# anthonyhu/tumblr-emotions

Hardware: AMD Instinct MI355X
Metric: training samples/sec (224x224 img + 32-tok text, batch 256) (higher is better)
Workload: dtype f32; 1 GPU; joint train step (fwd+bwd+all-reduce+Adam): Inception-v1 224x224x3 + 300-d embedding + LSTM-512, T=32, V=10000, 15 classes, batch 256 per GPU, reference freeze (<=Mixed_5b conv weights frozen, all BN betas trainable), dropout 0.8, BN train mode; global_batch=256, per_gpu_batch=256, parallelism=dp1, launch=eager

## Files before the change

### tumblr_emotions_amd/csrc/conv_igemm.hip

```cpp
#include <stdlib.h>
#include <mutex>
#include <type_traits>
#include <unordered_map>
#include "conv_epilogue.h"

using ds::f32x16;
typedef float f32x4 __attribute__((ext_vector_type(4)));
typedef float f32x2 __attribute__((ext_vector_type(2)));
typedef unsigned int u32x4 __attribute__((ext_vector_type(4)));
typedef __attribute__((address_space(3))) void *lds_ptr;

namespace {

constexpr int BK = 16;
constexpr int LDK = 20;
using ds::kOOB;
using ds::make_srd;

struct ConvParams {
    ds_conv_desc d;
    const float *x;
    const float *w;
    float *z;
    const float *bias;
// ... 772 lines not shown
                                                       srd_w, (okn && kk + 1 < d.Cin) ? (off + (unsigned)d.w_k_stride) * 4u : kOOB, 0, 0));
            }
        } else {
#pragma unroll
            for (int i = 0; i < BJ; ++i) {
                const int nn = n0 + srow + 32 * i;
                const bool ok = nn < d.Cout && k < d.Cin;
                const unsigned off = wt + (unsigned)nn * (unsigned)d.w_n_stride + (unsigned)k;
                rb[i] = __builtin_bit_cast(f32x4, __builtin_amdgcn_raw_buffer_load_b128(srd_w, ok ? off * 4u : kOOB, 0, 0));
            }
        }
        ++tap;
        if (++dw == d.KW) {
            dw = 0;
            if (++dh == d.KH) { dh = 0; tap = 0; c0 += HK; }
        }
    };

    auto store_tile = [&](int buf) {
        __bf16 *a_s = As + buf * BM * HLD;
        __bf16 *b_s = Bs + buf * BN * HLD;
#pragma unroll
        for (int j = 0; j < AJ; ++j)
            *reinterpret_cast<bf16x4 *>(a_s + (srow + 32 * j) * HLD + c4) = __builtin_convertvector(ra[j], bf16x4);
        if (BNMAJOR) {
#pragma unroll
            for (int i = 0; i < BP; ++i) {
                const int pi = tid + 256 * i;
                const int kp = pi / (BN / 4), n4 = pi - kp * (BN / 4);
                if (pi < 4 * BN) {
#pragma unroll
                    for (int jj = 0; jj < 4; ++jj) {
                        const f32x2 pr = {rb[2 * i][jj], rb[2 * i + 1][jj]};
                        *reinterpret_cast<bf16x2 *>(b_s + (4 * n4 + jj) * HLD + 2 * kp) = __builtin_convertvector(pr, bf16x2);
                    }
                }
            }
        } else {
#pragma unroll
            for (int i = 0; i < BJ; ++i)
                *reinterpret_cast<bf16x4 *>(b_s + (srow + 32 * i) * HLD + c4) = __builtin_convertvector(rb[i], bf16x4);
        }
    };

    auto compute = [&](int buf) {
        const __bf16 *a_s = As + buf * BM * HLD + (wm * 32 + li) * HLD + kh * 8;
        const __bf16 *b_s = Bs + buf * BN * HLD + li * HLD + kh * 8;
#pragma unroll
        for (int ks = 0; ks < 2; ++ks) {
            const bf16x8 a = *reinterpret_cast<const bf16x8 *>(a_s + ks * 16);
#pragma unroll
            for (int b = 0; b < NT; ++b) {
                const bf16x8 w = *reinterpret_cast<const bf16x8 *>(b_s + b * 32 * HLD + ks * 16);
                acc[b] = __builtin_amdgcn_mfma_f32_32x32x16_bf16(a, w, acc[b], 0, 0, 0);
            }
        }
    };

    int par = 0;
    if (tid0.row < p.row_tiles) {
        setup_tile(tid0.row);
        load_tile();
        store_tile(0);
    }
    __syncthreads();
    for (int tile = tid0.row; tile < p.row_tiles; tile += tid0.stride) {
        const int m0 = tile * BM;
        const bool has_next = tile + tid0.stride < p.row_tiles;
#pragma unroll
        for (int b = 0; b < NT; ++b)
#pragma unroll
            for (int r = 0; r < 16; ++r) acc[b][r] = 0.f;
        for (int kt = 0; kt < KT; ++kt) {
            const bool last = kt + 1 == KT;
            if (last && has_next) setup_tile(tile + tid0.stride);
            const bool fetch = !last || has_next;
            if (fetch) load_tile();
            compute(par);
            if (fetch) store_tile(par ^ 1);
            __syncthreads();
            par ^= 1;
        }
#pragma unroll
        for (int b = 0; b < NT; ++b) {
            const int col = n0 + b * 32 + li;
            const bool colok = col < d.Cout;
            const float bv = ((flags & DS_EPI_BIAS) && colok) ? p.bias[col] : 0.f;
            const float pv = (p.pivot && colok) ? p.pivot[col] : 0.f;
            float s = 0.f, q = 0.f;
#pragma unroll
            for (int r = 0; r < 16; ++r) {
                const int row = m0 + wm * 32 + (r & 3) + 8 * (r >> 2) + 4 * kh;
                if (row < p.M && colok) {
                    float v = acc[b][r] + bv;
                    const int64_t off = (int64_t)row * d.ldz + col;
                    if (flags & DS_EPI_ACCUM) v += zout[off];
                    if (flags & DS_EPI_MASK) v = p.mask[(int64_t)row * d.ldmask + col] > 0.f ? v : 0.f;
                    if (flags & DS_EPI_RELU) v = fmaxf(v, 0.f);
                    zout[off] = v;
                    const float u = v - pv;
                    s += u;
                    q += u * u;
                }
            }
            csum[b] += s;
            csq[b] += q;
        }
    }

    if (flags & DS_EPI_STATS) {
        float *red = reinterpret_cast<float *>(smem);
        __syncthreads();
#pragma unroll
        for (int b = 0; b < NT; ++b) {
            const float s = csum[b] + __shfl_xor(csum[b], 32);
            const float q = csq[b] + __shfl_xor(csq[b], 32);
            if (kh == 0) {
                const int c = b * 32 + li;
                red[(wm * BN + c) * 2 + 0] = s;
                red[(wm * BN + c) * 2 + 1] = q;
            }
        }
        __syncthreads();
        if (tid < BN && n0 + tid < d.Cout && tid0.row < p.row_tiles) {
            float s = 0.f, q = 0.f;
#pragma unroll
            for (int w = 0; w < 4; ++w) {
                s += red[(w * BN + tid) * 2 + 0];
                q += red[(w * BN + tid) * 2 + 1];
            }
            p.stats[(int64_t)(n0 + tid) * tid0.stride + tid0.row] = s;
            p.stats[((int64_t)d.Cout + n0 + tid) * tid0.stride + tid0.row] = q;
        }
    }
}


#ifndef DS_WIDE_A_B2B
#define DS_WIDE_A_B2B 1
#endif
template <int N>
__device__ __forceinline__ void barrier_keep_vm() { asm volatile("s_waitcnt vmcnt(%0) lgkmcnt(0)\n\ts_barrier" ::"n"(N) : "memory"); }

template <bool BNR>
struct WideEpi : ds::WaveRowOpt { static constexpr bool bnr = BNR, mask_rstd = true, publish = true; };

template <int NB, bool BNMAJOR, bool BNB = false, bool POOL = false, int AST = 0, bool BNR = false>
__global__ __launch_bounds__(256, NB <= 4 ? 3 : 2) void gemm_wide_kernel(const ConvParams p) {
    constexpr int BN = NB * 32, WK = 16;
    constexpr int DJ = (WK * BN / 4 + 255) / 256;
    constexpr int BSZ = DJ * 1024;
    constexpr int BST = AST > 0 ? AST - 1 : 2;
    static_assert(AST == 0 || (AST >= 3 && !BNB && !POOL), "the A ring is built for the plain and the normalising loader");
    __shared__ __attribute__((aligned(128))) float smem[BST * BSZ + 256 + AST * 2048];
    __shared__ __attribute__((aligned(16))) float nrm[BNB ? 5 : 2][1024 + WK];
    const ds_conv_desc &d = p.d;
    const int tid = threadIdx.x, lane = tid & 63;
    const int wave = __builtin_amdgcn_readfirstlane(tid >> 6);
    const int li = lane & 31, kh = lane >> 5;
    const TileId t0 = tile_id(p);
    const int n0 = t0.col * BN;
    const bool item = t0.row < p.row_tiles;
    const __amdgpu_buffer_rsrc_t srd_x = make_srd(p.x, p.x_bytes);
    const __amdgpu_buffer_rsrc_t srd_w = make_srd(p.w, p.w_bytes);
    const int K = d.Cin;
    int mrow0 = t0.row * 128 + wave * 32, Mw = p.M;
    bool hasU = false, hasD = false, hasL = false, hasR = false;
    int prow = 0;
    if constexpr (POOL) {
        const int blk = t0.row * 4 + wave;
        const int n = blk / p.pool_bpi, rb = blk - n * p.pool_bpi;
        const int r0 = rb * p.pool_rpb;
        const int rows = (d.H - r0) < p.pool_rpb ? (d.H - r0) : p.pool_rpb;
        const int cnt = (item && n < d.N) ? rows * d.W : 0;
        mrow0 = (n * d.H + r0) * d.W;
        Mw = mrow0 + cnt;
        const int dr = li / d.W, ow = li - dr * d.W, oh = r0 + dr;
        const bool ok = li < cnt;
        hasU = ok && oh > 0;
        hasD = ok && oh + 1 < d.H;
        hasL = ok && ow > 0;
        hasR = ok && ow + 1 < d.W;
        prow = d.W * d.ldx * 4;
    }
    const int m = mrow0 + li;
    const unsigned voff = (item && m < Mw) ? ((unsigned)m * (unsigned)d.ldx + 4u * kh) * 4u : kOOB;

    unsigned uoff[DJ];
    int ukq[DJ];
#pragma unroll
    for (int i = 0; i < DJ; ++i) {
        const int idx = i * 256 + tid;
        if (BNMAJOR) {
            const int k = idx / (BN / 4), n = n0 + (idx % (BN / 4)) * 4;
            ukq[i] = k;
            uoff[i] = (n < d.Cout && k < WK) ? ((unsigned)k * (unsigned)d.w_k_stride + (unsigned)n) * 4u : kOOB;
        } else {
            const int nl = idx >> 2, pc = idx & 3, kq = pc ^ ((nl >> 2) & 3);
            ukq[i] = kq * 4;
            uoff[i] = (n0 + nl < d.Cout && nl < BN) ? ((unsigned)(n0 + nl) * (unsigned)d.w_n_stride + 4u * kq) * 4u : kOOB;
        }
    }
    auto dma_b = [&](int buf, int c0, int i) {
        const bool ok = c0 + ukq[i] < K;
        const unsigned off = BNMAJOR ? uoff[i] + (unsigned)c0 * (unsigned)d.w_k_stride * 4u : uoff[i] + (unsigned)c0 * 4u;
        unsigned o = off;
        if (!ok || uoff[i] == 0x80000000u) o = 0x80000000u;
        __builtin_amdgcn_raw_ptr_buffer_load_lds(srd_w, (lds_ptr)(smem + buf * BSZ + wave * 256 + i * 1024), 16, o, 0, 0, 0);
    };

    f32x16 acc[NB];
#pragma unroll
    for (int b = 0; b < NB; ++b)
#pragma unroll
        for (int e = 0; e < 16; ++e) acc[b][e] = 0.f;

    const unsigned vup = (POOL && hasU) ? voff - (unsigned)prow : kOOB, vdn = (POOL && hasD) ? voff + (unsigned)prow : kOOB;
    const __amdgpu_buffer_rsrc_t srd_am = make_srd(POOL ? (const void *)d.pool_argmax : (const void *)p.x,
                                                   POOL ? (unsigned)((int64_t)p.M * K) : 0u);
    const unsigned vam = (POOL && item && m < Mw && t0.col == 0) ? (unsigned)m * (unsigned)K + 4u * kh : kOOB;
    f32x4 ru0, ru1, rd0, rd1;
    auto load_ud = [&](int c0) {
        ru0 = __builtin_bit_cast(f32x4, __builtin_amdgcn_raw_buffer_load_b128(srd_x, vup, c0 * 4, 0));
        ru1 = __builtin_bit_cast(f32x4, __builtin_amdgcn_raw_buffer_load_b128(srd_x, vup, c0 * 4 + 32, 0));
        rd0 = __builtin_bit_cast(f32x4, __builtin_amdgcn_raw_buffer_load_b128(srd_x, vdn, c0 * 4, 0));
        rd1 = __builtin_bit_cast(f32x4, __builtin_amdgcn_raw_buffer_load_b128(srd_x, vdn, c0 * 4 + 32, 0));
    };
    auto from_left = [](float v) -> float {
        return __builtin_bit_cast(float, __builtin_amdgcn_update_dpp(0, __builtin_bit_cast(int, v), 0x138 , 0xf, 0xf, false));
    };
    auto from_right = [](float v) -> float {
        return __builtin_bit_cast(float, __builtin_amdgcn_update_dpp(0, __builtin_bit_cast(int, v), 0x130 , 0xf, 0xf, false));
    };
    auto pool4 = [&](f32x4 &c, const f32x4 &u, const f32x4 &dn) -> unsigned {
        unsigned bytes = 0;
#pragma unroll
        for (int j = 0; j < 4; ++j) {
            const float uu = hasU ? u[j] : -INFINITY, dd = hasD ? dn[j] : -INFINITY;
            const float cm = fmaxf(fmaxf(uu, c[j]), dd);
            const int t = uu == cm ? 0 : (c[j] == cm ? 3 : 6);
            const float lraw = from_left(cm), rraw = from_right(cm);
            const int tl = __builtin_amdgcn_update_dpp(0, t, 0x138, 0xf, 0xf, false);
            const int tr = __builtin_amdgcn_update_dpp(0, t, 0x130, 0xf, 0xf, false);
            const float lv = hasL ? lraw : -INFINITY, rv = hasR ? rraw : -INFINITY;
            const float best = fmaxf(fmaxf(lv, cm), rv);
            const int il = lv == best ? tl : 99, ic = cm == best ? t + 1 : 99, ir = rv == best ? tr + 2 : 99;
            const int arg = min(min(il, ic), ir);
            c[j] = best;
            bytes |= (unsigned)arg << (8 * j);
        }
        return bytes;
    };
    f32x4 a0 = {0.f, 0.f, 0.f, 0.f}, a1 = {0.f, 0.f, 0.f, 0.f};
    if constexpr (AST == 0) {
        a0 = __builtin_bit_cast(f32x4, __builtin_amdgcn_raw_buffer_load_b128(srd_x, voff, 0, 0));
        a1 = __builtin_bit_cast(f32x4, __builtin_amdgcn_raw_buffer_load_b128(srd_x, voff, 32, 0));
    }
    if constexpr (POOL) load_ud(0);
    const ds_bn_bwd_on_load &bb = p.bnb;
    __amdgpu_buffer_rsrc_t srd_dy[3];
    unsigned vdy[3];
    if (BNB) {
#pragma unroll
        for (int sg = 0; sg < 3; ++sg) {
            const bool has = sg < bb.nseg;
            const int cb = sg == 0 ? 0 : bb.c_end[sg - 1];
            const int ld = has ? bb.ld[sg] : 0;
            srd_dy[sg] = make_srd(has ? bb.dy[sg] : bb.dy[0], has ? (unsigned)(((int64_t)(p.M - 1) * ld + (bb.c_end[sg] - cb)) * 4) : 0u);
            vdy[sg] = (has && item && m < p.M) ? ((unsigned)m * (unsigned)ld + 4u * kh) * 4u : kOOB;
        }
    }
    auto load_dy = [&](int c0, int half) -> f32x4 {
        const int sg = (c0 < bb.c_end[0] || bb.nseg == 1) ? 0 : ((c0 < bb.c_end[1] || bb.nseg == 2) ? 1 : 2);
        const int cb = sg == 0 ? 0 : bb.c_end[sg - 1];
        const __amdgpu_buffer_rsrc_t r = sg == 0 ? srd_dy[0] : (sg == 1 ? srd_dy[1] : srd_dy[2]);
        const unsigned v = sg == 0 ? vdy[0] : (sg == 1 ? vdy[1] : vdy[2]);
        return __builtin_bit_cast(f32x4, __builtin_amdgcn_raw_buffer_load_b128(r, v, (c0 - cb) * 4 + 32 * half, 0));
    };
    f32x4 d0 = {0.f, 0.f, 0.f, 0.f}, d1 = {0.f, 0.f, 0.f, 0.f};
    if (BNB) {
        d0 = load_dy(0, 0);
        d1 = load_dy(0, 1);
    }
    if constexpr (AST == 0) {
#pragma unroll
        for (int i = 0; i < DJ; ++i) dma_b(0, 0, i);
    }
    const int ksteps = (K + WK - 1) / WK;
    const bool norm = d.norm_rstd != nullptr;
    if (norm) {
        for (int c = tid; c < ksteps * WK; c += 256) {
            nrm[0][c] = c < K ? d.norm_rstd[c] : 0.f;
            nrm[1][c] = c < K ? d.norm_shift[c] : 0.f;
        }
    }
    auto apply_norm = [&](f32x4 &a, int c) {
        const f32x4 r = *reinterpret_cast<const f32x4 *>(&nrm[0][c]), sh = *reinterpret_cast<const f32x4 *>(&nrm[1][c]);
        const f32x4 zero = {0.f, 0.f, 0.f, 0.f};
        a = __builtin_elementwise_max(__builtin_elementwise_fma(a, r, sh), zero);
    };
    if (BNB) {
        for (int c = tid; c < ksteps * WK; c += 256) {
            nrm[0][c] = c < K ? bb.rstd[c] : 0.f;
            nrm[1][c] = c < K ? bb.shift[c] : 0.f;
            nrm[BNB ? 2 : 0][c] = c < K ? bb.mean[c] : 0.f;
            nrm[BNB ? 3 : 0][c] = c < K ? bb.coef[c] : 0.f;
            nrm[BNB ? 4 : 0][c] = c < K ? bb.coef[K + c] : 0.f;
        }
    }
    auto apply_bnb = [&](f32x4 &a, const f32x4 &dy, int c) {
        const f32x4 r = *reinterpret_cast<const f32x4 *>(&nrm[0][c]), sh = *reinterpret_cast<const f32x4 *>(&nrm[1][c]);
        const f32x4 mu = *reinterpret_cast<const f32x4 *>(&nrm[BNB ? 2 : 0][c]);
        const f32x4 k1 = *reinterpret_cast<const f32x4 *>(&nrm[BNB ? 3 : 0][c]), k2 = *reinterpret_cast<const f32x4 *>(&nrm[BNB ? 4 : 0][c]);
#pragma unroll
        for (int j = 0; j < 4; ++j) a[j] = ds::bn_bwd_dz(a[j], dy[j], r[j], sh[j], mu[j], k1[j], k2[j]);
    };
    __syncthreads();
    auto pool_step = [&](int c0) {
        const unsigned w0 = pool4(a0, ru0, rd0), w1 = pool4(a1, ru1, rd1);
        __builtin_amdgcn_raw_buffer_store_b32(w0, srd_am, vam, c0, 0);
        __builtin_amdgcn_raw_buffer_store_b32(w1, srd_am, vam, c0 + 8, 0);
    };
    if constexpr (POOL) pool_step(0);
    if (norm && AST == 0) {
        apply_norm(a0, 4 * kh);
        apply_norm(a1, 8 + 4 * kh);
    }
    if (BNB) {
        apply_bnb(a0, d0, 4 * kh);
        apply_bnb(a1, d1, 8 + 4 * kh);
    }
    if constexpr (AST > 0) {
        float *const ring = smem + BST * BSZ + 256;
        unsigned aoff[2];
#pragma unroll
        for (int j = 0; j < 2; ++j) {
            const int row = 16 * j + (lane >> 2), chunk = (lane & 3) ^ ((row >> 1) & 3);
            const int mr = mrow0 + row;
            aoff[j] = (item && mr < Mw) ? ((unsigned)mr * (unsigned)d.ldx + 4u * chunk) * 4u : kOOB;
        }
        auto dma_a = [&](int stage, int c0) {
#pragma unroll
            for (int j = 0; j < 2; ++j)
                __builtin_amdgcn_raw_ptr_buffer_load_lds(srd_x, (lds_ptr)(ring + (stage * 4 + wave) * 512 + j * 256), 16, aoff[j], c0 * 4, 0, 0);
        };
        auto dma_b_all = [&](int buf, int c0) {
#pragma unroll
            for (int i = 0; i < DJ; ++i) dma_b(buf, c0, i);
        };
#pragma unroll
        for (int j = -(AST - 1); j < 0; ++j) {
            if (j + AST - 2 >= 0 && j + AST - 2 < ksteps) dma_b_all((j + AST - 2) % BST, (j + AST - 2) * WK);
            if (j + AST - 1 < ksteps) dma_a((j + AST - 1) % AST, (j + AST - 1) * WK);
        }
        constexpr int KEEP = 2 * (AST - 2) + DJ * (AST - 3);
        if (ksteps > AST - 1) barrier_keep_vm<KEEP>(); else barrier_keep_vm<0>();
        int bst = 0, ast = 0;
        const int swz = (li >> 1) & 3;
        for (int ks = 0; ks < ksteps; ++ks) {
            const float *ra = ring + (ast * 4 + wave) * 512 + li * 16;
            a0 = *reinterpret_cast<const f32x4 *>(ra + ((kh ^ swz) * 4));
            a1 = *reinterpret_cast<const f32x4 *>(ra + (((2 + kh) ^ swz) * 4));
            if (norm) {
                apply_norm(a0, ks * WK + 4 * kh);
                apply_norm(a1, ks * WK + 8 + 4 * kh);
            }
            const float *b_s = smem + bst * BSZ;
#pragma unroll
            for (int b = 0; b < NB; ++b) {
                float bf[8];
                if (BNMAJOR) {
#pragma unroll
                    for (int j = 0; j < 4; ++j) {
                        bf[j] = b_s[(4 * kh + j) * BN + 32 * b + li];
                        bf[4 + j] = b_s[(8 + 4 * kh + j) * BN + 32 * b + li];
                    }
                } else {
                    const int nl = 32 * b + li, sw = (nl >> 2) & 3;
                    const f32x4 lo = *reinterpret_cast<const f32x4 *>(b_s + nl * 16 + ((kh ^ sw) * 4));
                    const f32x4 hi = *reinterpret_cast<const f32x4 *>(b_s + nl * 16 + (((2 + kh) ^ sw) * 4));
#pragma unroll
                    for (int j = 0; j < 4; ++j) { bf[j] = lo[j]; bf[4 + j] = hi[j]; }
                }
                if (b == 0) {
                    if (ks + AST - 2 < ksteps) dma_b_all((bst + AST - 2) % BST, (ks + AST - 2) * WK);
                    if (ks + AST - 1 < ksteps) dma_a((ast + AST - 1) % AST, (ks + AST - 1) * WK);
                }
                __builtin_amdgcn_sched_barrier(0);
#pragma unroll
                for (int j = 0; j < 4; ++j) acc[b] = __builtin_amdgcn_mfma_f32_32x32x2f32(a0[j], bf[j], acc[b], 0, 0, 0);
#pragma unroll
                for (int j = 0; j < 4; ++j) acc[b] = __builtin_amdgcn_mfma_f32_32x32x2f32(a1[j], bf[4 + j], acc[b], 0, 0, 0);
                __builtin_amdgcn_sched_barrier(0);
            }
            if (ks + AST - 1 < ksteps) barrier_keep_vm<KEEP>(); else barrier_keep_vm<0>();
            bst = bst + 1 == BST ? 0 : bst + 1;
            ast = ast + 1 == AST ? 0 : ast + 1;
        }
    }
    for (int ks = 0; AST == 0 && ks < ksteps; ++ks) {
        const bool more = ks + 1 < ksteps;
        const int cn = (ks + 1) * WK;
        const float *b_s = smem + (ks & 1) * BSZ;
        f32x4 n0v = a0, n1v = a1;
#pragma unroll
        for (int b = 0; b < NB; ++b) {
            float bf[8];
            if (BNMAJOR) {
#pragma unroll
                for (int j = 0; j < 4; ++j) {
                    bf[j] = b_s[(4 * kh + j) * BN + 32 * b + li];
                    bf[4 + j] = b_s[(8 + 4 * kh + j) * BN + 32 * b + li];
                }
            } else {
                const int nl = 32 * b + li, sw = (nl >> 2) & 3;
                const f32x4 lo = *reinterpret_cast<const f32x4 *>(b_s + nl * 16 + ((kh ^ sw) * 4));
                const f32x4 hi = *reinterpret_cast<const f32x4 *>(b_s + nl * 16 + (((2 + kh) ^ sw) * 4));
#pragma unroll
                for (int j = 0; j < 4; ++j) { bf[j] = lo[j]; bf[4 + j] = hi[j]; }
            }
            if (more) {
                if (b == 0) {
                    n0v = __builtin_bit_cast(f32x4, __builtin_amdgcn_raw_buffer_load_b128(srd_x, voff, cn * 4, 0));
                    if (BNB) d0 = load_dy(cn, 0);
                }
                if (b == ((NB > 1 && !DS_WIDE_A_B2B) ? 1 : 0)) {
                    n1v = __builtin_bit_cast(f32x4, __builtin_amdgcn_raw_buffer_load_b128(srd_x, voff, cn * 4 + 32, 0));
                    if (BNB) d1 = load_dy(cn, 1);
                    if constexpr (POOL) load_ud(cn);
                }
                if (b < DJ) dma_b((ks + 1) & 1, cn, b);
            }
            __builtin_amdgcn_sched_barrier(0);
#pragma unroll
            for (int j = 0; j < 4; ++j) acc[b] = __builtin_amdgcn_mfma_f32_32x32x2f32(a0[j], bf[j], acc[b], 0, 0, 0);
#pragma unroll
            for (int j = 0; j < 4; ++j) acc[b] = __builtin_amdgcn_mfma_f32_32x32x2f32(a1[j], bf[4 + j], acc[b], 0, 0, 0);
            __builtin_amdgcn_sched_barrier(0);
        }
        if (more && DJ > NB) {
#pragma unroll
            for (int i = NB; i < DJ; ++i) dma_b((ks + 1) & 1, cn, i);
        }
        a0 = n0v;
        a1 = n1v;
        if constexpr (POOL) {
            if (more) pool_step(cn);
        }
        if (norm && more) {
            apply_norm(a0, cn + 4 * kh);
            apply_norm(a1, cn + 8 + 4 * kh);
        }
        if (BNB && more) {
            apply_bnb(a0, d0, cn + 4 * kh);
            apply_bnb(a1, d1, cn + 8 + 4 * kh);
        }
        __syncthreads();
    }

    const int flags = d.flags;
    float *red = smem + BST * BSZ;
    ds::wave_row_epilogue<NB, WideEpi<BNR>>(acc, d, p.z, p.mask, p.stats, p.pivot, item, n0, mrow0, Mw, Mw > mrow0, t0.row, t0.stride,
                                            red, wave, li, kh, p.scale, p.shift, p.fin.ticket != nullptr);
    if (p.fin.ticket && item && (flags & DS_EPI_STATS)) {
        __builtin_amdgcn_s_waitcnt(0);
        __syncthreads();
        if (tid == 0) {
            const unsigned old = __hip_atomic_fetch_add(p.fin.ticket + t0.col, 1u, __ATOMIC_RELAXED, __HIP_MEMORY_SCOPE_AGENT);
            red[0] = old + 1 == (unsigned)p.row_tiles ? 1.f : 0.f;
        }
        __syncthreads();
        if (red[0] != 0.f) {
            const int cend = min(n0 + BN, d.Cout);
            for (int c = n0 + wave; c < cend; c += 4)
                ds::bn_finalize_channel_by_wave(p.stats, t0.stride, d.Cout, c, p.fin_inv_count, p.fin, p.pivot);
            if (tid == 0) __hip_atomic_store(p.fin.ticket + t0.col, 0u, __ATOMIC_RELAXED, __HIP_MEMORY_SCOPE_AGENT);
        }
    }
}


struct Bf16dEpi : ds::WaveRowOpt { static constexpr bool half = true, mask_rstd = true; };

template <int NB, int KS, bool XB, bool X3 = false>
__global__ __launch_bounds__(256, 2) void conv_bf16d_kernel(const ConvParams p) {
    constexpr int BN = NB * 32, SI = !X3 ? 4 : NB == 1 ? 4 : NB <= 4 ? 2 : 1, TAPS = KS * KS;
    constexpr int PL = X3 ? 3 : 1;
    constexpr int NSL = SI * PL * NB / 4;
    static_assert(SI * PL * NB % 4 == 0, "a step's weight tile must be whole 256-lane DMA instructions");
    constexpr int BSZ = SI * PL * BN * 16;
    static_assert(!(X3 && XB), "ds_conv_f32x3 reads fp32 activations");
    __shared__ __attribute__((aligned(128))) __bf16 smem[2 * BSZ + 512];
    __shared__ __attribute__((aligned(16))) float nrm[2][X3 ? 1024 + 16 : 4];
    const ds_conv_desc &d = p.d;
    const int tid = threadIdx.x, lane = tid & 63;
    const int wave = __builtin_amdgcn_readfirstlane(tid >> 6);
    const int li = lane & 31, kh = lane >> 5;
    const TileId t0 = tile_id(p);
    const int n0 = t0.col * BN;
    const bool item = t0.row < p.row_tiles;
    const __amdgpu_buffer_rsrc_t srd_x = make_srd(p.x, p.x_bytes);
    const __amdgpu_buffer_rsrc_t srd_w = make_srd(p.w, p.w_bytes);
    const int chunks = (d.Cin + 15) >> 4;
    const int iters = chunks * TAPS;
    const int nsteps = (iters + SI - 1) / SI;

    const int m = t0.row * 128 + wave * 32 + li;
    const bool rv = item && m < p.M;
    const int ohw = d.OH * d.OW;
    const int n = (rv ? m : 0) / ohw;
    const int r = (rv ? m : 0) - n * ohw;
    const int oh = r / d.OW, ow = r - oh * d.OW;
    unsigned voff[TAPS];
#pragma unroll
    for (int a = 0; a < KS; ++a)
#pragma unroll
        for (int b = 0; b < KS; ++b) {
            const int ih = oh * d.stride - d.pad_t + a, iw = ow * d.stride - d.pad_l + b;
            const bool ok = rv && (unsigned)ih < (unsigned)d.H && (unsigned)iw < (unsigned)d.W;
            voff[a * KS + b] = ok ? ((unsigned)((n * d.H + ih) * d.W + iw) * (unsigned)d.ldx + 8u * kh) * (XB ? 2u : 4u) : kOOB;
        }
    const int ncols = p.col_total;
    unsigned uoff[NSL];
    int uit[NSL];
#pragma unroll
    for (int i = 0; i < NSL; ++i) {
        const int sl = i * 256 + tid;
        const int itl = sl / (BN * 2), nn = (sl >> 1) % BN, half = sl & 1;
        uit[i] = itl;
        uoff[i] = (n0 + nn < ncols) ? ((unsigned)((itl * ncols + n0 + nn) * 16 + 8 * half)) * 2u : kOOB;
    }
    const unsigned it_bytes = (unsigned)ncols * 32u;
    auto dma_b = [&](int buf, int step, int i) {
        unsigned o = uoff[i] + (unsigned)(step * SI * PL) * it_bytes;
        if (step * SI * PL + uit[i] >= iters * PL || uoff[i] == 0x80000000u) o = 0x80000000u;
        __builtin_amdgcn_raw_ptr_buffer_load_lds(srd_w, (lds_ptr)(smem + buf * BSZ + wave * 512 + i * 2048), 16, o, 0, 0, 0);
    };
    auto load_a = [&](int it, f32x4 &lo, f32x4 &hi) {
        const int chunk = it / TAPS, tap = it - chunk * TAPS;
        unsigned vo = voff[0];
#pragma unroll
        for (int k = 1; k < TAPS; ++k) vo = tap == k ? voff[k] : vo;
        if (XB) {
            lo = __builtin_bit_cast(f32x4, __builtin_amdgcn_raw_buffer_load_b128(srd_x, vo, chunk * 32, 0));
        } else {
            lo = __builtin_bit_cast(f32x4, __builtin_amdgcn_raw_buffer_load_b128(srd_x, vo, chunk * 64, 0));
            hi = __builtin_bit_cast(f32x4, __builtin_amdgcn_raw_buffer_load_b128(srd_x, vo, chunk * 64 + 16, 0));
        }
    };

    f32x16 acc[NB];
#pragma unroll
    for (int b = 0; b < NB; ++b)
#pragma unroll
        for (int e = 0; e < 16; ++e) acc[b][e] = 0.f;

    f32x4 alo[SI], ahi[SI];
#pragma unroll
    for (int j = 0; j < SI; ++j) load_a(j, alo[j], ahi[j]);
#pragma unroll
    for (int i = 0; i < NSL; ++i) dma_b(0, 0, i);
    bool norm = false;
    if constexpr (X3) {
        norm = d.norm_rstd != nullptr;
        if (norm)
            for (int c = tid; c < chunks * 16; c += 256) {
                nrm[0][c] = c < d.Cin ? d.norm_rstd[c] : 0.f;
                nrm[1][c] = c < d.Cin ? d.norm_shift[c] : 0.f;
            }
    }
    __syncthreads();
    for (int st = 0; st < nsteps; ++st) {
        const bool more = st + 1 < nsteps;
        const __bf16 *b_s = smem + (st & 1) * BSZ + li * 16 + kh * 8;
        f32x4 nlo[SI], nhi[SI];
#pragma unroll
        for (int j = 0; j < SI; ++j) {
            bf16x8 af, af1, af2;
            if (XB) {
                af = __builtin_bit_cast(bf16x8, alo[j]);
            } else {
                f32x4 xl = alo[j], xh = ahi[j];
                if constexpr (X3) {
                    if (norm) {
                        const int c = ((st * SI + j) / TAPS) * 16 + 8 * kh;
                        const f32x4 zero = {0.f, 0.f, 0.f, 0.f};
                        xl = __builtin_elementwise_max(__builtin_elementwise_fma(xl, *reinterpret_cast<const f32x4 *>(&nrm[0][c]),
                                                                                 *reinterpret_cast<const f32x4 *>(&nrm[1][c])), zero);
                        xh = __builtin_elementwise_max(__builtin_elementwise_fma(xh, *reinterpret_cast<const f32x4 *>(&nrm[0][c + 4]),
                                                                                 *reinterpret_cast<const f32x4 *>(&nrm[1][c + 4])), zero);
                    }
                }
                bf16x4 l4 = __builtin_convertvector(xl, bf16x4), h4 = __builtin_convertvector(xh, bf16x4);
                af = __builtin_shufflevector(l4, h4, 0, 1, 2, 3, 4, 5, 6, 7);
                if constexpr (X3) {
                    xl -= __builtin_convertvector(l4, f32x4);
                    xh -= __builtin_convertvector(h4, f32x4);
                    l4 = __builtin_convertvector(xl, bf16x4);
                    h4 = __builtin_convertvector(xh, bf16x4);
                    af1 = __builtin_shufflevector(l4, h4, 0, 1, 2, 3, 4, 5, 6, 7);
                    xl -= __builtin_convertvector(l4, f32x4);
                    xh -= __builtin_convertvector(h4, f32x4);
                    af2 = __builtin_shufflevector(__builtin_convertvector(xl, bf16x4), __builtin_convertvector(xh, bf16x4), 0, 1, 2, 3, 4, 5, 6, 7);
                }
            }
            if (more) {
                load_a((st + 1) * SI + j, nlo[j], nhi[j]);
#pragma unroll
                for (int i = j; i < NSL; i += SI) dma_b((st + 1) & 1, st + 1, i);
            }
// ... 68 lines not shown
        const __bf16 p1 = (__bf16)r1;
        const __bf16 p2 = (__bf16)(r1 - (float)p1);
        const int64_t o = (((int64_t)it * 3) * ncols + col) * 16 + j;
        wb[o] = p0;
        wb[o + (int64_t)ncols * 16] = p1;
        wb[o + (int64_t)ncols * 32] = p2;
    }
}

typedef void (*KernelFn)(const ConvParams);

int64_t conv_M(const ds_conv_desc *d) { return (int64_t)d->N * d->OH * d->OW; }

template <int LO, int HI, class F>
KernelFn with_const(int i, F &&f) {
    if constexpr (LO < HI)
        if (i > LO) return with_const<LO + 1, HI>(i, f);
    return f(std::integral_constant<int, LO>{});
}

struct Tuning {
    int wide = 1;
    int wide_cost = 0;
    int wide_nb = 0;
    int wide_min_wgs = 128;
    int wide_ring = 0;
    int mt = 0, nt = 0;
    int path = 0;
    int prio = 0;
    int xcd_remap = 1;
    int bf16d_max_nb = 8;
};

Tuning &tuning() {
    static Tuning tune = [] {
        Tuning t;
        const auto knob = [](const char *name, int *v) {
            if (const char *e = ds::tune_env(name)) *v = atoi(e);
        };
        knob("DS_CONV_WIDE", &t.wide);
        knob("DS_WIDE_COST", &t.wide_cost);
        knob("DS_WIDE_NB", &t.wide_nb);
        knob("DS_WIDE_MINWGS", &t.wide_min_wgs);
        knob("DS_WIDE_RING", &t.wide_ring);
        knob("DS_CONV_PRIO", &t.prio);
        knob("DS_CONV_XCD_REMAP", &t.xcd_remap);
        if (const char *e = ds::tune_env("DS_CONV_CFG")) sscanf(e, "%d,%d", &t.mt, &t.nt);
        if (const char *e = ds::tune_env("DS_CONV_PATH")) t.path = e[0] == 'l' ? 1 : (e[0] == 'd' ? 2 : (e[0] == 'g' ? 3 : 0));
        return t;
    }();
    return tune;
}

struct TileCfg {
    int mt, nt;
    bool direct;
    bool glds;
    bool bf16;
    int wide;
};

struct Variant {
    bool bnmajor, fold, vec;
};

enum Ask { kAsIs, kBeforeBnb, kBeforePool };

struct Launch {
    Variant v;
    TileCfg c;
    bool bnr, pool, bnb;
    int row_tiles, gx, gy;
    bool one;
    dim3 grid;
    int col_tiles;
    int partials;
};

bool dims_vec(const ds_conv_desc *d) {
    const bool bnmajor = d->w_n_stride == 1 && d->w_k_stride != 1;
    const bool a_vec = (d->ldx % 4 == 0) && (d->Cin % 4 == 0);
    const bool b_vec = bnmajor ? (d->Cout % 4 == 0) && (d->w_k_stride % 4 == 0) && (d->w_tap_stride % 4 == 0)
                               : (d->Cin % 4 == 0) && (d->w_n_stride % 4 == 0) && (d->w_tap_stride % 4 == 0);
    return a_vec && b_vec;
}

bool aligned16(const void *x, const void *w) { return (((uintptr_t)x | (uintptr_t)w) & 15) == 0; }

KernelFn kernel_of(const Launch &L) {
    const TileCfg &c = L.c;
    const Variant &v = L.v;
    if (c.wide) {
        if (L.bnr) {
            if (L.pool)
                return with_const<1, 4>(c.wide, [](auto nb) { return gemm_wide_kernel<decltype(nb)::value, true, false, true, 0, true>; });
            return with_const<1, 8>(c.wide, [](auto nb) { return gemm_wide_kernel<decltype(nb)::value, true, false, false, 0, true>; });
        }
        if (L.pool)
            return with_const<1, 4>(c.wide, [](auto nb) { return gemm_wide_kernel<decltype(nb)::value, true, false, true>; });
        if (L.bnb)
            return with_const<1, 2>(c.wide, [](auto nb) { return gemm_wide_kernel<decltype(nb)::value, false, true>; });
#ifdef DS_TUNING
        const int ring = tuning().wide_ring;
        if ((ring == 3 || ring == 4) && c.wide >= 2 && c.wide <= 4)
            return with_const<2, 4>(c.wide, [&](auto nb) {
                return with_const<3, 4>(ring, [&](auto ast) {
                    return v.bnmajor ? gemm_wide_kernel<decltype(nb)::value, true, false, false, decltype(ast)::value>
                                     : gemm_wide_kernel<decltype(nb)::value, false, false, false, decltype(ast)::value>;
                });
            });
#endif
        return with_const<1, 8>(c.wide, [&](auto nb) {
            return v.bnmajor ? gemm_wide_kernel<decltype(nb)::value, true> : gemm_wide_kernel<decltype(nb)::value, false>;
        });
    }
    if (L.bnr) {
        if (c.glds) return with_const<1, 3>(c.nt, [](auto nt) { return conv_glds_kernel<decltype(nt)::value, true, true>; });
        return with_const<1, 6>(c.nt, [](auto nt) { return conv_igemm_kernel<1, decltype(nt)::value, true, false, true, true>; });
    }
    if (c.bf16)
        return with_const<1, 4>(c.nt, [&](auto nt) {
            constexpr int NT = decltype(nt)::value;
            if (v.fold) return conv_bf16_kernel<NT, true, true>;
            return v.bnmajor ? conv_bf16_kernel<NT, true, false> : conv_bf16_kernel<NT, false, false>;
        });
    if (c.glds)
        return with_const<1, 3>(c.nt, [&](auto nt) {
            return v.bnmajor ? conv_glds_kernel<decltype(nt)::value, true> : conv_glds_kernel<decltype(nt)::value, false>;
        });
    return with_const<1, 2>(c.mt == 2 ? 2 : 1, [&](auto mt) {
        constexpr int MT = decltype(mt)::value;
        if (c.direct)
            return with_const<1, 4>(c.nt, [&](auto nt) {
                constexpr int NT = decltype(nt)::value;
                if (v.bnmajor) return v.fold ? conv_direct_kernel<MT, NT, true, true> : conv_direct_kernel<MT, NT, true, false>;
                return conv_direct_kernel<MT, NT, false, false>;
            });
        return with_const<1, 6>(c.nt, [&](auto nt) {
            constexpr int NT = decltype(nt)::value;
            if (v.bnmajor) {
                if (v.fold) return conv_igemm_kernel<MT, NT, true, true, true>;
                return v.vec ? conv_igemm_kernel<MT, NT, true, false, true> : conv_igemm_kernel<MT, NT, true, false, false>;
            }
            return v.vec ? conv_igemm_kernel<MT, NT, false, false, true> : conv_igemm_kernel<MT, NT, false, false, false>;
        });
    });
}

int pool3_nb(const ds_conv_desc *d, bool vec) {
    if (!vec || d->dtype != DS_DTYPE_F32) return 0;
    if (d->KH != 1 || d->KW != 1 || d->stride != 1 || d->fold_cin || d->splits > 1 || d->bnb) return 0;
    if (d->flags & ~(DS_EPI_STATS | DS_EPI_BN_RELU)) return 0;
    if (!(d->w_n_stride == 1 && d->w_k_stride != 1)) return 0;
    if (d->W > 32 || d->Cin % 16 != 0 || d->Cin < 32 || d->Cin > 1024 || d->Cout > 128) return 0;
    const int64_t M = conv_M(d);
    if (((M - 1) * d->ldz + d->Cout) * 4 >= (1ll << 31) || M * d->Cin >= (1ll << 31)) return 0;
    return (d->Cout + 31) / 32;
}

void pool3_blocks(const ds_conv_desc *d, int *rpb, int *bpi) {
    *rpb = 32 / d->W;
    *bpi = (d->H + *rpb - 1) / *rpb;
}

int wide_nb(const ds_conv_desc *d, bool vec, Ask ask) {
    if (d->pool_argmax || ask == kBeforePool) return pool3_nb(d, vec);
    const Tuning &t = tuning();
    if (!t.wide || !vec || d->dtype != DS_DTYPE_F32) return 0;
    if (d->KH != 1 || d->KW != 1 || d->stride != 1 || d->fold_cin || d->splits > 1) return 0;
    if (d->flags & ~(DS_EPI_STATS | DS_EPI_ACCUM | DS_EPI_BNSUMS | DS_EPI_BN_RELU)) return 0;
    if (d->Cin % 8 != 0 || d->Cin < 32) return 0;
    const int64_t M = conv_M(d);
    if (((M - 1) * d->ldz + d->Cout) * 4 >= (1ll << 31)) return 0;
    if ((d->flags & DS_EPI_BNSUMS) && ((M - 1) * d->ldmask + d->Cout) * 4 >= (1ll << 31)) return 0;
    const int N = d->Cout;
    int best = 0, best_pad = 0;
    int64_t best_cost = (int64_t)1 << 60;
    const int64_t row_tiles = (M + 127) / 128;
    const int nb_max = (d->bnb || ask == kBeforeBnb) ? 2 : 8;
    for (int nb = nb_max; nb >= (N <= 32 ? 1 : 2); --nb) {
        const int tiles = (N + 32 * nb - 1) / (32 * nb);
        const int64_t rounds = (row_tiles * tiles + ds::kCUs - 1) / ds::kCUs;
        const int64_t cost = rounds * (2 * nb + t.wide_cost);
        if (cost < best_cost) { best_cost = cost; best = nb; best_pad = tiles * 32 * nb; }
    }
    if (t.wide_nb >= 1 && t.wide_nb <= nb_max) {
        best = t.wide_nb;
        best_pad = (N + 32 * best - 1) / (32 * best) * 32 * best;
    }
    const int64_t wgs = row_tiles * ((N + 32 * best - 1) / (32 * best));
    if (t.wide < 2 && (wgs < t.wide_min_wgs || best_pad * 100 > N * 125)) return 0;
    return best;
}

int resident_per_cu(KernelFn kernel) {
    static std::unordered_map<const void *, int> cache;
    static std::mutex guard;
    const std::lock_guard<std::mutex> lock(guard);
    int &slot = cache[(const void *)kernel];
    if (slot == 0) {
        int n = 0;
        if (hipOccupancyMaxActiveBlocksPerMultiprocessor(&n, (const void *)kernel, 256, 0) != hipSuccess || n < 1) n = 1;
        slot = n > 8 ? 8 : n;
    }
    return slot;
}

TileCfg pick_cfg(const ds_conv_desc *d, bool vec, Ask ask) {
    const Tuning &t = tuning();
    const int64_t M = conv_M(d);
    const int N = d->Cout;
    const int pad32 = (N + 31) / 32 * 32, pad64 = (N + 63) / 64 * 64;
    TileCfg c = {1, 1, false, false, false, 0};
    if (int nb = wide_nb(d, vec, ask)) {
        c.wide = nb;
        c.nt = nb;
        return c;
    }
    if (d->dtype == DS_DTYPE_BF16) {
        c.bf16 = true;
        int best = 4, best_pad = 1 << 30;
        for (int nt = 4; nt >= 2; --nt) {
            const int pad = (N + 32 * nt - 1) / (32 * nt) * (32 * nt);
            if (pad < best_pad) { best_pad = pad; best = nt; }
        }
        c.nt = N <= 32 ? 1 : best;
        if (d->tile_nt > 0) c.nt = d->tile_nt > 4 ? 4 : d->tile_nt;
        if (t.nt > 0) c.nt = t.nt > 4 ? 4 : t.nt;
        return c;
    }
    c.direct = vec && t.path == 2;
    if (c.direct) {
        const int64_t row_tiles = (M + 31) / 32;
        if (pad64 * 100 <= pad32 * 112 && row_tiles * (pad64 / 64) >= 12 * ds::kCUs) c.nt = 2;
    } else {
        const int64_t row_tiles = (M + 127) / 128;
        if (pad64 * 100 <= pad32 * 112 && row_tiles * (pad64 / 64) >= 5 * ds::kCUs / 2) c.nt = 2;
    }
    if (d->tile_nt > 0 && !c.direct) c.nt = d->tile_nt > 6 ? 6 : d->tile_nt;
    if (t.mt > 0) c.mt = t.mt;
    if (t.nt > 0) c.nt = t.nt;
    if (c.direct && c.nt > 4) c.nt = 4;
    if (!c.direct && vec && d->fold_cin == 0 && t.path != 1) {
        const int k16 = (d->Cin + 15) / 16 * 16, k32 = (d->Cin + 31) / 32 * 32;
        if (t.path == 3 || (d->KH * d->KW >= 4 && k32 * 100 <= k16 * 112)) {
            c.glds = true;
            c.mt = 1;
            if (c.nt > 3) c.nt = 3;
        }
    }
    return c;
}

constexpr int kOneTilePerWg = 2048;

Launch choose(const ds_conv_desc *d, bool aligned, Ask ask = kAsIs) {
    Launch L;
    L.v = {d->w_n_stride == 1 && d->w_k_stride != 1, d->fold_cin > 0, dims_vec(d) && aligned};
    const TileCfg c = L.c = pick_cfg(d, L.v.vec, ask);
    L.bnr = false;
    L.pool = d->pool_argmax || ask == kBeforePool;
    L.bnb = d->bnb != nullptr;
    const int bm = (c.direct ? 32 : 128) * (c.glds ? 1 : c.mt), bn = 32 * c.nt;
    L.row_tiles = (int)((conv_M(d) + bm - 1) / bm);
    if (c.wide && L.pool) {
        int rpb, bpi;
        pool3_blocks(d, &rpb, &bpi);
        L.row_tiles = (int)(((int64_t)d->N * bpi + 3) / 4);
    }
    L.gy = (d->Cout + bn - 1) / bn;
    const int wg_tiles = c.direct ? (L.row_tiles + 3) / 4 : L.row_tiles;
    L.gx = wg_tiles;
    L.one = true;
    if (!c.wide && (wg_tiles > kOneTilePerWg || c.direct)) {
        int target = (resident_per_cu(kernel_of(L)) * ds::kCUs) / L.gy;
        if (target < 8) target = 8;
        L.gx = wg_tiles < target ? wg_tiles : target;
        if (L.gx >= 8) L.gx &= ~7;
        L.one = false;
    }
    if (d->grid_x > 0 && !c.direct) {
        L.gx = d->grid_x < wg_tiles ? d->grid_x : wg_tiles;
        L.one = L.gx == wg_tiles;
    }
    L.bnr = (d->flags & DS_EPI_BN_RELU) != 0;
    L.grid = dim3(L.gx, L.gy, d->splits > 1 ? d->splits : 1);
    L.col_tiles = 0;
    if (L.one && (c.wide || (tuning().xcd_remap && L.gy > 1)) && !c.direct) {
        L.col_tiles = L.gy;
        L.grid = dim3((L.row_tiles * L.gy + 7) / 8 * 8, 1, L.grid.z);
    }
    L.partials = c.direct ? L.gx * 4 : L.gx;
    return L;
}

bool bnr_ok(const ds_conv_desc *d, const Launch &L) {
    if (d->dtype != DS_DTYPE_F32 || !L.v.bnmajor || !L.v.vec || L.v.fold || d->splits > 1 || d->bnb || d->fin) return false;
    return !L.c.bf16 && !L.c.direct && L.c.mt == 1;
}

int fill_params(ConvParams &p, const char *who, const char *hint, const ds_conv_desc *d, const void *x, const void *w, float *z,
                const void *mask, float *stats, const float *pivot, int64_t prepared_w_bytes = -1) {
    p = ConvParams{};
    p.d = *d;
    if (d->splits <= 1) p.d.z_split_stride = 0;
    p.x = (const float *)x; p.w = (const float *)w; p.z = z; p.mask = (const float *)mask; p.stats = stats;
    p.pivot = (d->flags & DS_EPI_STATS) ? pivot : nullptr;
// ... 334 lines not shown
```

Baseline: 20190 samples/s.

## Stage pool input tile in LDS to share 3x3 neighbors across waves

The fused maxpool-before-1x1-conv path now stages each block's input channel slice in a double-buffered, swizzled LDS tile. Up and down neighbours are read from that tile instead of being reloaded from global memory. Only the first and last waves fetch halo rows, and the argmax bytes are packed into a single 64-bit store via permlane32 swap. This cuts redundant global loads for the pooling stencil at the cost of extra LDS space, a barrier per K step and more index logic. The eligibility check is also relaxed to allow Cin of 16.

```diff
diff --git a/tumblr_emotions_amd/csrc/conv_igemm.hip b/tumblr_emotions_amd/csrc/conv_igemm.hip
--- a/tumblr_emotions_amd/csrc/conv_igemm.hip
+++ b/tumblr_emotions_amd/csrc/conv_igemm.hip
@@ -948,7 +948,8 @@
     constexpr int BSZ = DJ * 1024;
     constexpr int BST = AST > 0 ? AST - 1 : 2;
     static_assert(AST == 0 || (AST >= 3 && !BNB && !POOL), "the A ring is built for the plain and the normalising loader");
-    __shared__ __attribute__((aligned(128))) float smem[BST * BSZ + 256 + AST * 2048];
+    constexpr int PT = 2048;
+    __shared__ __attribute__((aligned(128))) float smem[BST * BSZ + 256 + AST * 2048 + (POOL ? 2 * PT : 0)];
     __shared__ __attribute__((aligned(16))) float nrm[BNB ? 5 : 2][1024 + WK];
     const ds_conv_desc &d = p.d;
     const int tid = threadIdx.x, lane = tid & 63;
@@ -963,6 +964,8 @@
     int mrow0 = t0.row * 128 + wave * 32, Mw = p.M;
     bool hasU = false, hasD = false, hasL = false, hasR = false;
     int prow = 0;
+    bool upM = false, dnM = false;
+    int pu = 0, pd = 0;
     if constexpr (POOL) {
         const int blk = t0.row * 4 + wave;
         const int n = blk / p.pool_bpi, rb = blk - n * p.pool_bpi;
@@ -978,6 +981,14 @@
         hasL = ok && ow > 0;
         hasR = ok && ow + 1 < d.W;
         prow = d.W * d.ldx * 4;
+        const bool top = dr == 0, bot = dr + 1 == rows;
+        upM = hasU && top && wave == 0;
+        dnM = hasD && bot && wave == 3;
+        pu = pd = wave * 32 + li;
+        if (hasU && !top) pu -= d.W;
+        if (hasU && top && wave > 0) pu = (wave - 1) * 32 + (p.pool_rpb - 1) * d.W + ow;
+        if (hasD && !bot) pd += d.W;
+        if (hasD && bot && wave < 3) pd = (wave + 1) * 32 + ow;
     }
     const int m = mrow0 + li;
     const unsigned voff = (item && m < Mw) ? ((unsigned)m * (unsigned)d.ldx + 4u * kh) * 4u : kOOB;
@@ -1011,16 +1022,37 @@
 #pragma unroll
         for (int e = 0; e < 16; ++e) acc[b][e] = 0.f;
 
-    const unsigned vup = (POOL && hasU) ? voff - (unsigned)prow : kOOB, vdn = (POOL && hasD) ? voff + (unsigned)prow : kOOB;
+    const unsigned vup = (POOL && upM) ? voff - (unsigned)prow : kOOB, vdn = (POOL && dnM) ? voff + (unsigned)prow : kOOB;
     const __amdgpu_buffer_rsrc_t srd_am = make_srd(POOL ? (const void *)d.pool_argmax : (const void *)p.x,
                                                    POOL ? (unsigned)((int64_t)p.M * K) : 0u);
-    const unsigned vam = (POOL && item && m < Mw && t0.col == 0) ? (unsigned)m * (unsigned)K + 4u * kh : kOOB;
-    f32x4 ru0, ru1, rd0, rd1;
-    auto load_ud = [&](int c0) {
-        ru0 = __builtin_bit_cast(f32x4, __builtin_amdgcn_raw_buffer_load_b128(srd_x, vup, c0 * 4, 0));
-        ru1 = __builtin_bit_cast(f32x4, __builtin_amdgcn_raw_buffer_load_b128(srd_x, vup, c0 * 4 + 32, 0));
-        rd0 = __builtin_bit_cast(f32x4, __builtin_amdgcn_raw_buffer_load_b128(srd_x, vdn, c0 * 4, 0));
-        rd1 = __builtin_bit_cast(f32x4, __builtin_amdgcn_raw_buffer_load_b128(srd_x, vdn, c0 * 4 + 32, 0));
+    const unsigned vam = (POOL && item && m < Mw && t0.col == 0) ? (unsigned)m * (unsigned)K + 8u * kh : kOOB;
+    const bool halo = POOL && (wave == 0 || wave == 3);
+    const unsigned vhalo = wave == 0 ? vup : vdn;
+    f32x4 rh0 = {0.f, 0.f, 0.f, 0.f}, rh1 = {0.f, 0.f, 0.f, 0.f};
+    auto load_halo = [&](int c0) {
+        if (halo) {
+            rh0 = __builtin_bit_cast(f32x4, __builtin_amdgcn_raw_buffer_load_b128(srd_x, vhalo, c0 * 4, 0));
+            rh1 = __builtin_bit_cast(f32x4, __builtin_amdgcn_raw_buffer_load_b128(srd_x, vhalo, c0 * 4 + 32, 0));
+        }
+    };
+    float *const ptile = smem + BST * BSZ + 256;
+    const int pown = wave * 32 + li, sown = (li >> 1) & 3, sup = (pu >> 1) & 3, sdn = (pd >> 1) & 3;
+    unsigned vco[2] = {kOOB, kOOB};
+    int tco[2] = {0, 0};
+    if constexpr (POOL) {
+#pragma unroll
+        for (int j = 0; j < 2; ++j) {
+            const int row = 16 * j + (lane >> 2), chunk = lane & 3;
+            vco[j] = (item && mrow0 + row < Mw) ? ((unsigned)(mrow0 + row) * (unsigned)d.ldx + 4u * chunk) * 4u : kOOB;
+            tco[j] = (wave * 32 + row) * 16 + ((chunk ^ ((row >> 1) & 3)) * 4);
+        }
+    }
+    auto tile_put = [&](int st, const f32x4 &c0v, const f32x4 &c1v) {
+        *reinterpret_cast<f32x4 *>(ptile + st * PT + tco[0]) = c0v;
+        *reinterpret_cast<f32x4 *>(ptile + st * PT + tco[1]) = c1v;
+    };
+    auto tile_get = [&](int st, int px, int sw, int half) -> f32x4 {
+        return *reinterpret_cast<const f32x4 *>(ptile + st * PT + px * 16 + (((2 * half + kh) ^ sw) * 4));
     };
     auto from_left = [](float v) -> float {
         return __builtin_bit_cast(float, __builtin_amdgcn_update_dpp(0, __builtin_bit_cast(int, v), 0x138 , 0xf, 0xf, false));
@@ -1048,11 +1080,13 @@
         return bytes;
     };
     f32x4 a0 = {0.f, 0.f, 0.f, 0.f}, a1 = {0.f, 0.f, 0.f, 0.f};
+    const unsigned va0 = POOL ? vco[0] : voff, va1 = POOL ? vco[1] : voff;
+    constexpr int kA1 = POOL ? 0 : 32;
     if constexpr (AST == 0) {
-        a0 = __builtin_bit_cast(f32x4, __builtin_amdgcn_raw_buffer_load_b128(srd_x, voff, 0, 0));
-        a1 = __builtin_bit_cast(f32x4, __builtin_amdgcn_raw_buffer_load_b128(srd_x, voff, 32, 0));
-    }
-    if constexpr (POOL) load_ud(0);
+        a0 = __builtin_bit_cast(f32x4, __builtin_amdgcn_raw_buffer_load_b128(srd_x, va0, 0, 0));
+        a1 = __builtin_bit_cast(f32x4, __builtin_amdgcn_raw_buffer_load_b128(srd_x, va1, kA1, 0));
+    }
+    if constexpr (POOL) load_halo(0);
     const ds_bn_bwd_on_load &bb = p.bnb;
     __amdgpu_buffer_rsrc_t srd_dy[3];
     unsigned vdy[3];
@@ -1111,13 +1145,37 @@
 #pragma unroll
         for (int j = 0; j < 4; ++j) a[j] = ds::bn_bwd_dz(a[j], dy[j], r[j], sh[j], mu[j], k1[j], k2[j]);
     };
+    if constexpr (POOL) tile_put(0, a0, a1);
     __syncthreads();
-    auto pool_step = [&](int c0) {
-        const unsigned w0 = pool4(a0, ru0, rd0), w1 = pool4(a1, ru1, rd1);
-        __builtin_amdgcn_raw_buffer_store_b32(w0, srd_am, vam, c0, 0);
-        __builtin_amdgcn_raw_buffer_store_b32(w1, srd_am, vam, c0 + 8, 0);
-    };
-    if constexpr (POOL) pool_step(0);
+    f32x4 pn0 = {0.f, 0.f, 0.f, 0.f}, pn1 = {0.f, 0.f, 0.f, 0.f};
+    auto pool_step = [&](int c0, int st, int cnext) {
+        if (cnext >= 0) {
+            pn0 = __builtin_bit_cast(f32x4, __builtin_amdgcn_raw_buffer_load_b128(srd_x, va0, cnext * 4, 0));
+            pn1 = __builtin_bit_cast(f32x4, __builtin_amdgcn_raw_buffer_load_b128(srd_x, va1, cnext * 4, 0));
+        }
+        a0 = tile_get(st, pown, sown, 0);
+        a1 = tile_get(st, pown, sown, 1);
+        f32x4 u0 = tile_get(st, pu, sup, 0), u1 = tile_get(st, pu, sup, 1);
+        f32x4 e0 = tile_get(st, pd, sdn, 0), e1 = tile_get(st, pd, sdn, 1);
+        if (halo) {
+            if (wave == 0) {
+                u0 = upM ? rh0 : u0;
+                u1 = upM ? rh1 : u1;
+            } else {
+                e0 = dnM ? rh0 : e0;
+                e1 = dnM ? rh1 : e1;
+            }
+        }
+        __builtin_amdgcn_sched_barrier(0);
+        if (cnext >= 0) load_halo(cnext);
+        __builtin_amdgcn_sched_barrier(0);
+        const unsigned w0 = pool4(a0, u0, e0), w1 = pool4(a1, u1, e1);
+        const auto sw = __builtin_amdgcn_permlane32_swap(w0, w1, false, false);
+        typedef unsigned u32x2 __attribute__((ext_vector_type(2)));
+        const u32x2 pr = {sw[0], sw[1]};
+        __builtin_amdgcn_raw_buffer_store_b64(pr, srd_am, vam, c0, 0);
+    };
+    if constexpr (POOL) pool_step(0, 0, ksteps > 1 ? WK : -1);
     if (norm && AST == 0) {
         apply_norm(a0, 4 * kh);
         apply_norm(a1, 8 + 4 * kh);
@@ -1216,14 +1274,13 @@
                 for (int j = 0; j < 4; ++j) { bf[j] = lo[j]; bf[4 + j] = hi[j]; }
             }
             if (more) {
-                if (b == 0) {
+                if (b == 0 && !POOL) {
                     n0v = __builtin_bit_cast(f32x4, __builtin_amdgcn_raw_buffer_load_b128(srd_x, voff, cn * 4, 0));
                     if (BNB) d0 = load_dy(cn, 0);
                 }
-                if (b == ((NB > 1 && !DS_WIDE_A_B2B) ? 1 : 0)) {
+                if (b == ((NB > 1 && !DS_WIDE_A_B2B) ? 1 : 0) && !POOL) {
                     n1v = __builtin_bit_cast(f32x4, __builtin_amdgcn_raw_buffer_load_b128(srd_x, voff, cn * 4 + 32, 0));
                     if (BNB) d1 = load_dy(cn, 1);
-                    if constexpr (POOL) load_ud(cn);
                 }
                 if (b < DJ) dma_b((ks + 1) & 1, cn, b);
             }
@@ -1238,10 +1295,13 @@
 #pragma unroll
             for (int i = NB; i < DJ; ++i) dma_b((ks + 1) & 1, cn, i);
         }
-        a0 = n0v;
-        a1 = n1v;
         if constexpr (POOL) {
-            if (more) pool_step(cn);
+            if (more) tile_put((ks + 1) & 1, pn0, pn1);
+            __syncthreads();
+            if (more) pool_step(cn, (ks + 1) & 1, ks + 2 < ksteps ? cn + WK : -1);
+        } else {
+            a0 = n0v;
+            a1 = n1v;
         }
         if (norm && more) {
             apply_norm(a0, cn + 4 * kh);
@@ -1251,7 +1311,7 @@
             apply_bnb(a0, d0, cn + 4 * kh);
             apply_bnb(a1, d1, cn + 8 + 4 * kh);
         }
-        __syncthreads();
+        if constexpr (!POOL) __syncthreads();
     }
 
     const int flags = d.flags;
@@ -1626,7 +1686,7 @@
     if (d->KH != 1 || d->KW != 1 || d->stride != 1 || d->fold_cin || d->splits > 1 || d->bnb) return 0;
     if (d->flags & ~(DS_EPI_STATS | DS_EPI_BN_RELU)) return 0;
     if (!(d->w_n_stride == 1 && d->w_k_stride != 1)) return 0;
-    if (d->W > 32 || d->Cin % 16 != 0 || d->Cin < 32 || d->Cin > 1024 || d->Cout > 128) return 0;
+    if (d->W > 32 || d->Cin % 16 != 0 || d->Cin < 16 || d->Cin > 1024 || d->Cout > 128) return 0;
     const int64_t M = conv_M(d);
     if (((M - 1) * d->ldz + d->Cout) * 4 >= (1ll << 31) || M * d->Cin >= (1ll << 31)) return 0;
     return (d->Cout + 31) / 32;
```

Measured after the change: 20500 samples/s, median of 6. 1.02x the previous value.
